# olof3/QuantumOptimalControl.jl

Hardware: AMD Instinct MI355X
Metric: GRAPE gradient evals/sec (dim N, T slices, B seeds) @ 1/2/4/8 GPU (higher is better)
Workload: dtype f64

## Files before the change

quantumoptimalcontrol.jl_amd/csrc/qoc_blkseg.hpp:

```cpp
#pragma once
#include "qoc_blku.hpp"

namespace qoc {

struct BlksegParams {
  double rad[3];
  double mur[3], mui[3];
  double theta_cap;
  int S;
  int L;
  int UPW;
  int RB;
  const double* u;
  double* u_copy;
  double* u_copy2;
  double* J2;
  cx<double>* coef2;
  double* dJdu;
  unsigned long long* terms;
  unsigned int* done;
  double* best;
  long long seed_offset;
  double* best_res;
  double* best_out;
  double2* gseg;
  const int* stale;
  const double2* gtab;
  double pen_mu;
  unsigned int prow[3];
  unsigned int pcol;
  double2* dseg;
};
enum { BLKSEG_FUSED = 0, BLKSEG_FWD = 1, BLKSEG_BWD = 2 };

__host__ __device__ inline size_t blkseg_off_rec(int NB, int nblk) { return (size_t)6 * NB * NB * nblk; }
__host__ __device__ inline size_t blkseg_off_slot(int NB, int nblk, int Nt) { return blkseg_off_rec(NB, nblk) + 4 * (size_t)Nt; }
__host__ __device__ inline size_t blkseg_off_g0(int NB, int nblk, int Nt, int S) {
  return blkseg_off_slot(NB, nblk, Nt) + (size_t)2 * S * NB * NB * nblk;
}
__host__ __device__ inline size_t blkseg_off_xN(int NB, int nblk, int Nt, int S) {
  return blkseg_off_g0(NB, nblk, Nt, S) + (size_t)2 * NB * NB * nblk;
}
__host__ __device__ inline size_t blkseg_off_xt(int N, int m, int NB, int nblk, int Nt, int S) {
  return blkseg_off_xN(NB, nblk, Nt, S) + (size_t)2 * N * m;
}
__host__ __device__ inline size_t blkseg_off_cf(int N, int m, int NB, int nblk, int Nt, int S) {
  return blkseg_off_xt(N, m, NB, nblk, Nt, S) + (size_t)2 * N * m;
}
__host__ __device__ inline size_t blkseg_off_red(int N, int m, int NB, int nblk, int Nt, int S) {
  return blkseg_off_cf(N, m, NB, nblk, Nt, S) + (size_t)4 * m;
}
__host__ __device__ inline size_t blkseg_off_wred(int N, int m, int NB, int nblk, int Nt, int S) {
  return blkseg_off_red(N, m, NB, nblk, Nt, S) + 32;
}
__host__ __device__ inline size_t blkseg_off_dJ(int N, int m, int NB, int nblk, int Nt, int S, int W, int RB) {
  return blkseg_off_wred(N, m, NB, nblk, Nt, S) + (size_t)128 * W * RB;
}
__host__ __device__ inline size_t blkseg_off_d0(int N, int m, int nu, int NB, int nblk, int Nt, int S, int W, int RB) {
  return (blkseg_off_dJ(N, m, NB, nblk, Nt, S, W, RB) + (size_t)Nt * nu + 1) & ~(size_t)1;
}
__host__ __device__ inline size_t blkseg_lds(int N, int m, int nu, int NB, int nblk, int Nt, int S, int W, int RB,
                                             bool pen = false) {
  if (pen) return (blkseg_off_d0(N, m, nu, NB, nblk, Nt, S, W, RB) + (size_t)2 * NB * NB * nblk) * sizeof(double);
  return (blkseg_off_dJ(N, m, NB, nblk, Nt, S, W, RB) + (size_t)Nt * nu) * sizeof(double);
}
constexpr size_t BLKSEG_LDS_MAX = (size_t)160 * 1024;
__host__ __device__ inline int blkseg_rb(int upw, int nu) {
  const int r = 64 / (upw * (nu > 0 ? nu : 1));
  return r < 1 ? 1 : r > 4 ? 4 : r;
}

#ifdef QOC_PROBE
static __device__ unsigned long long g_segw[32];
#define SEGW_SET(slot, v)                                                        \
  do {                                                                           \
    if (blockIdx.x == 7 && (threadIdx.x & 63) == 0) g_segw[slot] = (v);          \
  } while (0)
static __device__ int g_seg_noturn, g_seg_turnmode;
#define SEG_TURNS (!g_seg_noturn)
#define SEG_TURNMODE g_seg_turnmode
#else
#define SEG_TURNS true
#define SEG_TURNMODE 1
#define SEGW_SET(slot, v) \
  do {                    \
  } while (0)
#endif


template <int NB, bool AH, bool BH>
__device__ __forceinline__ void seg_mm(const double (&ar)[NB * NB], const double (&ai)[NB * NB], const double (&br)[NB * NB],
                                       const double (&bi)[NB * NB], double (&cr)[NB * NB], double (&ci)[NB * NB]) {
#pragma unroll
  for (int i = 0; i < NB; ++i)
#pragma unroll
    for (int k = 0; k < NB; ++k) {
      double sr = 0.0, si = 0.0;
#pragma unroll
      for (int q = 0; q < NB; ++q) {
        const int ea = AH ? q * NB + i : i * NB + q, eb = BH ? k * NB + q : q * NB + k;
// ... 207 lines not shown
#pragma unroll
  for (int k = K - 1; k >= 0; --k) {
    ct = fma(ct, t2, T.c[k]);
    st = fma(st, t2, T.s[k]);
  }
  st *= t;
}
template <int K = BLKSEG_KMAX>
__device__ __forceinline__ void sk2_z(const Sk2& g0, const double* rec, double& zr, double& zi) {
  double ct, st;
  sk2_phase<K>(g0.d0, g0.d1, ct, st);
  const double2 ph = *reinterpret_cast<const double2*>(rec);
  zr = ph.x * ct - ph.y * st;
  zi = fma(ph.x, st, ph.y * ct);
}
template <int K = BLKSEG_KMAX, bool EX = false>
__device__ __forceinline__ void sk2_form(const Sk2 (&g)[3], double2 ph, double2 u, Sk2& ah, double (&ur)[4],
                                         double (&ui)[4], double* ex = nullptr) {
  constexpr BlksegTrig T = blkseg_trig();
  ah.d0 = fma(u.y, g[2].d0, fma(u.x, g[1].d0, g[0].d0));
  ah.d1 = fma(u.y, g[2].d1, fma(u.x, g[1].d1, g[0].d1));
  ah.r = fma(u.y, g[2].r, fma(u.x, g[1].r, g[0].r));
  ah.q = fma(u.y, g[2].q, fma(u.x, g[1].q, g[0].q));
  const double a = 0.5 * (ah.d0 - ah.d1);
  const double w = fma(a, a, fma(ah.r, ah.r, ah.q * ah.q));
  double cw = T.c[K], sw = T.s[K], s3 = EX ? T.d[K] : 0.0, ct, st;
#pragma unroll
  for (int k = K - 1; k >= 0; --k) {
    cw = fma(cw, w, T.c[k]);
    sw = fma(sw, w, T.s[k]);
// ... 385 lines not shown
  constexpr int NV1 = NB == 2 ? 2 : 1;
  const int N = g.N, m = g.m, nu = g.nu, Nt = g.Nt, nblk = bk.nblk, S = sp.S, L = sp.L;
  const int tid = threadIdx.x, nthr = blockDim.x, w = tid >> 6, l = tid & 63, W = nthr >> 6;
  const int b = blockIdx.x;
  const size_t Nm = (size_t)N * m;
  BK_T(t0);
  double* const lds = reinterpret_cast<double*>(smem);
  double2* const gsh = reinterpret_cast<double2*>(lds);
  double* const rec = lds + blkseg_off_rec(NB, nblk);
  double2* const slot = reinterpret_cast<double2*>(lds + blkseg_off_slot(NB, nblk, Nt));
  double2* const g0s = reinterpret_cast<double2*>(lds + blkseg_off_g0(NB, nblk, Nt, S));
  double* const xN = lds + blkseg_off_xN(NB, nblk, Nt, S);
  double2* const xtl = reinterpret_cast<double2*>(lds + blkseg_off_xt(N, m, NB, nblk, Nt, S));
  cx<double>* const cf = reinterpret_cast<cx<double>*>(lds + blkseg_off_cf(N, m, NB, nblk, Nt, S));
  double* const red = lds + blkseg_off_red(N, m, NB, nblk, Nt, S);
  double* const wred = lds + blkseg_off_wred(N, m, NB, nblk, Nt, S);
  const int RB = sp.RB;
  double* const dJ = lds + blkseg_off_dJ(N, m, NB, nblk, Nt, S, W, RB);
  double2* const d0s = reinterpret_cast<double2*>(lds + blkseg_off_d0(N, m, nu, NB, nblk, Nt, S, W, RB));

  const int uw = l / nblk;
  const bool lact = uw < sp.UPW;
  const int beta = lact ? l - uw * nblk : 0;
  int pm = 0;
  if constexpr (PEN) {
    if (lact && w * sp.UPW + uw < S)
#pragma unroll
      for (int i = 0; i < NB; ++i) pm |= (int)((sp.prow[i] >> beta) & 1u) << i;
  }
  constexpr int PE = PEN ? NB * NB : 1;
  const int ntab = 3 * E * nblk;
  const double2* const x0g = reinterpret_cast<const double2*>(g.x0) + (g.x0_per_seed ? (size_t)b * Nm : 0);
  const double2* const xtg = reinterpret_cast<const double2*>(g.Xt);
  const double* ub = sp.u + (size_t)b * Nt * nu;
  const bool u16 = nu == 2 && (reinterpret_cast<size_t>(ub) & 15) == 0;
  auto load_u = [&](int k) -> double2 {
    if (u16) return reinterpret_cast<const double2*>(ub)[k];
    return make_double2(nu > 0 ? ub[(size_t)k * nu] : 0.0, nu > 1 ? ub[(size_t)k * nu + 1] : 0.0);
  };
  const bool hasx = MODE != BLKSEG_BWD && (size_t)tid < Nm;
  double2 tab0 = make_double2(0.0, 0.0), x00 = tab0, xt0 = tab0, ua = tab0, ubb = tab0;
  if (tid < ntab) tab0 = sp.gtab[tid];
  if (hasx) {
    x00 = x0g[tid];
    xt0 = xtg[tid];
  }
  if (tid < Nt) ua = load_u(tid);
  if (tid + nthr < Nt) ubb = load_u(tid + nthr);
  int brw[NB];
#pragma unroll
  for (int i = 0; i < NB; ++i) brw[i] = bk.brow[beta * NB + i];
  {
    if (tid < ntab) gsh[tid] = tab0;
    for (int q = tid + nthr; q < ntab; q += nthr) gsh[q] = sp.gtab[q];
    if constexpr (MODE != BLKSEG_BWD) {
      double2* const xN2 = reinterpret_cast<double2*>(xN);
      if (hasx) {
        xN2[tid] = x00;
        xtl[tid] = xt0;
      }
      for (size_t o = (size_t)tid + nthr; o < Nm; o += nthr) {
        xN2[o] = x0g[o];
        xtl[o] = xtg[o];
      }
    }
  }
  double rmax = 0.0;
  const bool cmu = sp.mur[1] == 0.0 && sp.mur[2] == 0.0 && sp.mui[1] == 0.0 && sp.mui[2] == 0.0;
  double2 emu0 = make_double2(1.0, 0.0);
  if (cmu) {
    const double er = exp(sp.mur[0]);
    double sn, cs;
    sincos(sp.mui[0], &sn, &cs);
    emu0 = make_double2(er * cs, er * sn);
  }
  auto slice = [&](int k, double2 uk) {
    const double u1 = uk.x, u2 = uk.y;
    for (int j = 0; j < nu; ++j) {
      const double v = j ? u2 : u1;
      if (sp.u_copy) sp.u_copy[((size_t)b * Nt + k) * nu + j] = v;
      if (sp.u_copy2) sp.u_copy2[((size_t)b * Nt + k) * nu + j] = v;
    }
    rmax = fmax(rmax, fma(fabs(u2), sp.rad[2], fma(fabs(u1), sp.rad[1], sp.rad[0])));
    double2* r = reinterpret_cast<double2*>(rec + 4 * (size_t)k);
    if (cmu) {
      r[0] = emu0;
    } else {
      const double mr = fma(u2, sp.mur[2], fma(u1, sp.mur[1], sp.mur[0]));
      const double mi = fma(u2, sp.mui[2], fma(u1, sp.mui[1], sp.mui[0]));
      const double er = exp(mr);
      double sn, cs;
      sincos(mi, &sn, &cs);
      r[0] = make_double2(er * cs, er * sn);
    }
    r[1] = make_double2(u1, u2);
  };
  if (tid < Nt) slice(tid, ua);
  if (tid + nthr < Nt) slice(tid + nthr, ubb);
  for (int k = tid + 2 * nthr; k < Nt; k += nthr) slice(k, load_u(k));
  rmax = block_max(rmax, red);
  int J = 0;
  double s0 = 1.0;
  while (rmax * s0 > sp.theta_cap && J < 60) {
    s0 *= 0.5;
    ++J;
  }
  int P = 0;
  {
    const double bb = rmax * s0, tol = 1.1102230246251565e-16;
    constexpr BlkuCoef K = blku_coef();
    double term = bb;
#pragma unroll
    for (int q = 0; q < BLKU_TMAX; ++q) {
      if (!(term > tol * fma(-bb, K.inv[q + 2], 1.0))) break;
      P = q + 1;
      term *= bb * K.inv[q + 2];
    }
  }
  P = __builtin_amdgcn_readfirstlane(P);
  J = __builtin_amdgcn_readfirstlane(J);
  int nex = 1;
  if constexpr (ORD == 0) nex = __builtin_amdgcn_readfirstlane(blkseg_exact_terms(rmax));
  if (tid < 8) reinterpret_cast<int*>(red + 24)[tid] = 0;
  if (J) {
    for (int k = tid; k < Nt; k += nthr) {
      rec[4 * (size_t)k + 2] *= s0;
      rec[4 * (size_t)k + 3] *= s0;
    }
  }
  __syncthreads();
  BK_T(t1);
  BK_ADD(0, t1 - t0);

  const int s = w * sp.UPW + uw;
  const bool sact = lact && s < S;
  const int kb = sact ? s * L : 0;
  const int ke = sact ? min(kb + L, Nt) : 0;
  double2 greg[GREG ? 3 : 1][GREG ? E : 1];
  if constexpr (GREG) {
#pragma unroll
    for (int j = 0; j < 3; ++j)
#pragma unroll
      for (int e = 0; e < E; ++e) greg[j][e] = gsh[(beta * 3 + j) * E + e];
  }
  auto gen_at = [&](int bc) {
    return [&, bc](int j, int e) -> double2 {
// ... 23 lines not shown
  double Hr[PE], Hi[PE];
#pragma unroll
  for (int e = 0; e < PE; ++e) Hr[e] = Hi[e] = 0.0;
  const int Lf = Nt - (S - 1) * L;
  const bool fast = NB == 2 && J == 0;
  Sk2 gk[3];
  if constexpr (NB == 2) {
#pragma unroll
    for (int j = 0; j < 3; ++j) {
      double2 e4[4];
#pragma unroll
      for (int e = 0; e < 4; ++e) e4[e] = gsh[(beta * 3 + j) * E + e];
      gk[j] = sk2_of(e4);
    }
  }
  const bool zdl = NB != 2 || (gk[1].d0 == 0.0 && gk[1].d1 == 0.0 && gk[2].d0 == 0.0 && gk[2].d1 == 0.0);
  const bool zd = __syncthreads_and(zdl ? 1 : 0) != 0 && cmu && sp.mur[0] == 0.0;
  const double za0 = NB == 2 ? 0.5 * (gk[0].d0 - gk[0].d1) : 0.0;
  const int ksel = __builtin_amdgcn_readfirstlane(blkseg_series_k(rmax * s0));
  const bool su = fast && zd;
  double pq[4] = {1.0, 0.0, 0.0, 0.0};
  auto lane_z = [&](double& zr, double& zi) {
    zr = 1.0;
    zi = 0.0;
    if constexpr (NB == 2) {
      if (su) {
        if (ksel == 5) sk2_z<5>(gk[0], rec, zr, zi);
        else if (ksel == 7) sk2_z<7>(gk[0], rec, zr, zi);
        else sk2_z<BLKSEG_KMAX>(gk[0], rec, zr, zi);
      }
    }
  };
  const double* const reck = rec + 4 * (size_t)kb;
  auto p1_fast = [&](int jj, auto SEL_, auto K_, auto ZD_) {
    constexpr bool SEL = decltype(SEL_)::value;
    constexpr int KS = decltype(K_)::value;
    constexpr bool ZD = decltype(ZD_)::value;
    if constexpr (NB == 2) {
    if constexpr (ZD) {
      double vv[2][4];
      bool act[2];
#pragma unroll
      for (int v = 0; v < 2; ++v) {
        const int k = kb + jj + v;
// ... 168 lines not shown
      ti[e] = v.y;
    }
    wave_lds_sync();
    if (take) {
      double cr[E], ci[E];
      seg_mm<NB, false, false>(qr, qi, tr, ti, cr, ci);
#pragma unroll
      for (int e = 0; e < E; ++e) {
        qr[e] = cr[e];
        qi[e] = ci[e];
        slot_at(s, e) = make_double2(cr[e], ci[e]);
      }
    }
    wave_lds_sync();
  }
  lds_barrier();
  if (sact && w > 0) {
    double er[E], ei[E];
#pragma unroll
    for (int e = 0; e < E; ++e) {
      const double2 v = slot_at(UPW - 1, e);
      er[e] = v.x;
      ei[e] = v.y;
    }
    for (int v = 1; v < w; ++v) {
      double tr[E], ti[E], cr[E], ci[E];
#pragma unroll
      for (int e = 0; e < E; ++e) {
        const double2 x = slot_at(v * UPW + UPW - 1, e);
        tr[e] = x.x;
        ti[e] = x.y;
      }
      seg_mm<NB, false, false>(tr, ti, er, ei, cr, ci);
#pragma unroll
      for (int e = 0; e < E; ++e) {
        er[e] = cr[e];
        ei[e] = ci[e];
      }
    }
    double cr[E], ci[E];
    seg_mm<NB, false, false>(qr, qi, er, ei, cr, ci);
#pragma unroll
    for (int e = 0; e < E; ++e) {
      qr[e] = cr[e];
      qi[e] = ci[e];
    }
  }
  if constexpr (PEN) {
    if (pm) {
      double tr[E], ti[E];
      seg_mm<NB, true, false>(qr, qi, Hr, Hi, tr, ti);
      seg_mm<NB, false, false>(tr, ti, qr, qi, Hr, Hi);
    }
  }
  const bool last = sact && s == S - 1;
  if (last) {
    double znr = 1.0, zni = 0.0;
    if (su) {
      double br, bi;
      lane_z(br, bi);
      for (int n = Nt; n > 0; n >>= 1) {
        if (n & 1) {
          const double t = znr * br - zni * bi;
          zni = fma(znr, bi, zni * br);
          znr = t;
        }
        const double t = br * br - bi * bi;
        bi = 2.0 * (br * bi);
        br = t;
      }
    }
    for (int c = 0; c < m; ++c) {
      double xr[NB], xi[NB];
#pragma unroll
      for (int i = 0; i < NB; ++i) {
        const size_t o = 2 * ((size_t)c * N + max(brw[i], 0));
        xr[i] = brw[i] >= 0 ? xN[o] : 0.0;
        xi[i] = brw[i] >= 0 ? xN[o + 1] : 0.0;
      }
#pragma unroll
      for (int i = 0; i < NB; ++i) {
        double yr = 0.0, yi = 0.0;
#pragma unroll
        for (int q = 0; q < NB; ++q) {
          yr = fma(qr[i * NB + q], xr[q], fma(-qi[i * NB + q], xi[q], yr));
          yi = fma(qr[i * NB + q], xi[q], fma(qi[i * NB + q], xr[q], yi));
        }
        if (su) {
          const double t = yr * znr - yi * zni;
          yi = fma(yr, zni, yi * znr);
          yr = t;
        }
        if (brw[i] >= 0) {
          const size_t o = 2 * ((size_t)c * N + brw[i]);
          xN[o] = yr;
          xN[o + 1] = yi;
        }
      }
    }
  }
  __syncthreads();
  if constexpr (PEN) {
    if (pm)
#pragma unroll
      for (int e = 0; e < E; ++e) slot_at(s, e) = make_double2(Hr[e], Hi[e]);
    wave_lds_sync();
    for (int d = 1; d < UPW; d <<= 1) {
      const bool take = pm && uw0 + d < UPW && s + d < S;
      double tr[E], ti[E];
#pragma unroll
      for (int e = 0; e < E; ++e) {
        const double2 v = take ? slot_at(s + d, e) : make_double2(0.0, 0.0);
        tr[e] = v.x;
        ti[e] = v.y;
      }
      wave_lds_sync();
// ... 48 lines not shown
  }
  if (tid == 0) {
    double Jv = red[16];
    if constexpr (PEN) {
      double ps = 0.0;
      for (int q = 0; q < nblk; ++q) ps += wred[q];
      Jv = fma(sp.pen_mu, ps, Jv);
    }
    __hip_atomic_store(reinterpret_cast<unsigned long long*>(g.J + b),
                       (unsigned long long)__double_as_longlong(Jv), __ATOMIC_RELAXED, __HIP_MEMORY_SCOPE_AGENT);
    if (sp.J2) sp.J2[b] = Jv;
  }
#if defined(__HIP_DEVICE_COMPILE__) && !defined(__gfx950__)
#error "k_blkseg_eval's best-(J, seed) hand-off is written for gfx950"
#endif
  const bool early = W <= 4;
  auto publish = [&]() {
    if (w != 0 || !sp.done) return;
    unsigned int prev = 0;
    if (l == 0) {
      asm volatile("s_waitcnt vmcnt(0)" ::: "memory");
      prev = __hip_atomic_fetch_add(sp.done, 1u, __ATOMIC_RELAXED, __HIP_MEMORY_SCOPE_AGENT);
    }
    prev = __shfl(prev, 0);
    if (prev == gridDim.x - 1) {
      __builtin_amdgcn_fence(__ATOMIC_ACQUIRE, "agent");
      asm volatile("s_waitcnt vmcnt(0)" ::: "memory");
      double bv = __builtin_inf();
      long long bi = -1;
      for (int e = l; e < (int)gridDim.x; e += 64) {
// ... 52 lines not shown
#pragma unroll
    for (int e = 0; e < E; ++e) g0s[e * nblk + beta] = make_double2(cr[e], ci[e]);
  }
  if constexpr (PEN) {
    if (pm) {
      later_waves(Hr, Hi);
      if (uw0 + 1 < UPW && s + 1 < S)
#pragma unroll
        for (int e = 0; e < E; ++e) {
          const double2 x = slot_at(s + 1, e);
          Hr[e] += x.x;
          Hi[e] += x.y;
        }
    }
  }
  __syncthreads();
  {
    double hr[E], hi[E], tr[E], ti[E];
#pragma unroll
    for (int e = 0; e < E; ++e) {
      const double2 v = g0s[e * nblk + beta];
      hr[e] = v.x;
      hi[e] = v.y;
    }
    if constexpr (PEN) {
      if (pm) {
        double dr[E], di[E];
#pragma unroll
        for (int e = 0; e < E; ++e) {
          const double2 v = d0s[e * nblk + beta];
          dr[e] = v.x;
// ... 23 lines not shown
#pragma unroll
            for (int q = 0; q < NB; ++q) {
              sr = fma(dr[i * NB + q], Hr[q * NB + j], fma(-di[i * NB + q], Hi[q * NB + j], sr));
              si = fma(dr[i * NB + q], Hi[q * NB + j], fma(di[i * NB + q], Hr[q * NB + j], si));
            }
            hr[i * NB + j] = fma(f, sr, hr[i * NB + j]);
            hi[i * NB + j] = fma(f, si, hi[i * NB + j]);
          }
        __builtin_amdgcn_sched_barrier(0);
      }
    }
    seg_mm<NB, false, false>(qr, qi, hr, hi, tr, ti);
    seg_mm<NB, false, true>(tr, ti, qr, qi, Gr, Gi);
  }

  if (!early) publish();
  BK_T(t2e);
  BK_ADD(2, t2e - t2);
  if constexpr (MODE == BLKSEG_FWD) {
    if (sact)
#pragma unroll
      for (int e = 0; e < E; ++e) gseg_at(e) = make_double2(Gr[e], Gi[e]);
    if (sp.terms && tid == 0) atomicAdd(sp.terms + b % TERM_SLOTS, (unsigned long long)Nt * ((unsigned long long)P << J));
    return;
  }
  }
  BK_T(t3);
  const double mu1r = sp.mur[1], mu1i = sp.mui[1], mu2r = sp.mur[2], mu2i = sp.mui[2];
  const double pen2 = PEN ? 2.0 * sp.pen_mu : 0.0;
  auto pen_step = [&](const double (&ur)[E], const double (&ui)[E]) {
    seg_pen_step<NB>(pm, pen2, slot + (size_t)opaque(s) * E * nblk + beta, nblk, ur, ui, Gr, Gi);
  };
  double zr, zi;
  lane_z(zr, zi);
  if (su) {
#pragma unroll
    for (int e = 0; e < E; ++e) {
      const double t = fma(zr, Gr[e], zi * Gi[e]);
      Gi[e] = fma(zr, Gi[e], -zi * Gr[e]);
      Gr[e] = t;
    }
  }
  const double pen2r = pen2 * zr, pen2i = -pen2 * zi;
  auto pen_step_v = [&](const double (&ur)[E], const double (&ui)[E]) {
    seg_pen_step<NB, true>(pm, pen2r, slot + (size_t)opaque(s) * E * nblk + beta, nblk, ur, ui, Gr, Gi, pen2i);
  };
  double* const wr = wred + 128 * RB * w;
  const int nrl = sp.UPW * max(nu, 1);
  const int rq = l / nrl, rrem = l - rq * nrl, ro = rrem / max(nu, 1), rj = rrem - ro * max(nu, 1);
  int rslot = 0;
  auto reduce = [&](int jj, double acc1, double acc2) {
    const int r = rslot;
    rslot = r == RB - 1 ? 0 : r + 1;
    *reinterpret_cast<double2*>(wr + 128 * r + 2 * l) = make_double2(acc1, acc2);
    if (r == RB - 1 || jj == 0) {
      wave_lds_sync();
      if (rq <= r) {
        const int ss = w * sp.UPW + ro, kk = ss * L + jj + r - rq;
        if (ss < S && kk < Nt) {
          const double* src = wr + 128 * rq + 2 * ro * nblk + rj;
          double sum = 0.0;
          for (int q = 0; q < nblk; ++q) sum += src[2 * q];
          dJ[(size_t)kk * nu + rj] = sum;
        }
      }
      wave_lds_sync();
    }
  };
  double pa1[4] = {0, 0, 0, 0}, pa2[4] = {0, 0, 0, 0};
  const double zxd0 = NB == 2 ? gk[0].d0 + sp.mui[0] : 0.0, zxd1 = NB == 2 ? gk[0].d1 + sp.mui[0] : 0.0;
  const double zx0 = 0.5 * (zxd0 + zxd1), zx3 = 0.5 * (zxd0 - zxd1), zx02 = zx0 * zx0;
  if constexpr (NB == 2) {
    sk2_pauli2(Sk2{gk[1].d0 + mu1i, gk[1].d1 + mu1i, gk[1].r, gk[1].q}, pa1);
    sk2_pauli2(Sk2{gk[2].d0 + mu2i, gk[2].d1 + mu2i, gk[2].r, gk[2].q}, pa2);
  }
  auto p3_fast = [&](int jj, auto SEL_, auto K_, auto ZD_, const double2* upre = nullptr) {
    constexpr bool SEL = decltype(SEL_)::value;
    constexpr int KS = decltype(K_)::value;
// ... 130 lines not shown
        const double2* const gp = slot + (size_t)opaque(sact ? s : 0) * E * nblk + beta;
#pragma unroll
        for (int e = 0; e < E; ++e) {
          const double2 v = gp[e * nblk];
          Gr[e] = v.x;
          Gi[e] = v.y;
        }
      }
      reduce(jj, act ? acc1 : 0.0, act ? acc2 : 0.0);
    }
  }
  if (turns || sprog.on) __builtin_amdgcn_s_setprio(0);
  BK_T(t4);
  BK_ADD(3, t4 - t3);
  SEGW_SET(16 + w, t4 - t0);
  __syncthreads();
  double* const og = sp.dJdu + (size_t)b * Nt * nu;
  for (int i = tid; i < Nt * nu; i += nthr) og[i] = dJ[i];
  if (MODE == BLKSEG_FUSED && sp.terms && tid == 0)
    atomicAdd(sp.terms + b % TERM_SLOTS, (unsigned long long)Nt * ((unsigned long long)P << J));
  BK_T(t5);
  BK_ADD(4, t5 - t4);
  BK_ADD(5, t5 - t0);
}

}
```

quantumoptimalcontrol.jl_amd/csrc/qoc_engine.hip:

```cpp
#include <dlfcn.h>

#include "qoc_internal.hpp"
#include "qoc_spline.hpp"
#include "qoc_opt.hpp"

namespace qoc_host {

thread_local std::string g_err;

int fail(qoc_ctx* ctx, int code, const char* fmt, ...) {
  char buf[512];
  va_list ap;
  va_start(ap, fmt);
  vsnprintf(buf, sizeof(buf), fmt, ap);
  va_end(ap);
  g_err = buf;
  if (ctx) ctx->err = buf;
  return code;
}

template <typename T>
int upload_complex(qoc_ctx* ctx, const double* host, void* dev, size_t nelem) {
  if (sizeof(T) == sizeof(double)) {
    HIPCHK(ctx, hipMemcpyAsync(dev, host, nelem * 16, hipMemcpyHostToDevice, ctx->stream));
// ... 483 lines not shown
  *out = c;
  return QOC_OK;
}

void qoc_destroy(qoc_ctx* c) {
  if (!c) return;
  hipSetDevice(c->dev);
  if (c->stream) hipStreamSynchronize(c->stream);
  if (c->comm && rccl().commDestroy) rccl().commDestroy(c->comm);
  if (c->d_best) hipFree(c->d_best);
  if (c->d_done) hipFree(c->d_done);
  if (c->d_tcoef) hipFree(c->d_tcoef);
  if (c->d_coef_mu) hipFree(c->d_coef_mu);
  if (c->d_brow) hipFree(c->d_brow);
  if (c->d_gtab) hipFree(c->d_gtab);
  if (c->d_wrow) hipFree(c->d_wrow);
  if (c->d_wrow_live) hipFree(c->d_wrow_live);
  if (c->d_dead_rows) hipFree(c->d_dead_rows);
  if (c->d_gc_part) hipFree(c->d_gc_part);
  if (c->d_gseg) hipFree(c->d_gseg);
  if (c->d_blkp_ctab) hipFree(c->d_blkp_ctab);
  if (c->d_blkp_M) hipFree(c->d_blkp_M);
  if (c->d_blkp_ph) hipFree(c->d_blkp_ph);
  if (c->d_minmax) hipFree(c->d_minmax);
  if (c->h_minmax) hipHostFree(c->h_minmax);
  if (c->h_flag) hipHostFree(c->h_flag);
  if (c->flag_ev) hipEventDestroy(c->flag_ev);
  void* ptrs[] = {c->d_A, c->d_x0, c->d_Xt, c->d_pmask, c->d_u,    c->d_U,    c->d_X, c->d_L, c->d_u_lam, c->d_coef_lam, c->d_blkU, c->d_J_scr, c->d_coef_scr,
                  c->d_J, c->d_coef, c->d_dJdu, c->d_flag, c->d_hist, c->d_stage, c->d_ws, c->d_red, c->d_Bs, c->d_cstage, c->d_fws, c->d_AH, c->d_Cst, c->d_gws, c->d_pws, c->d_ps, c->d_At, c->d_steps, c->d_terms, c->d_src, c->d_rsec, c->d_sink, c->d_blkrec, c->d_xn};
  for (void* p : ptrs)
// ... 1271 lines not shown
```

quantumoptimalcontrol.jl_amd/csrc/qoc_internal.hpp:

```cpp
#pragma once
#include <hip/hip_runtime.h>

#include <algorithm>
#include <cmath>
#include <cstdarg>
#include <cstdio>
#include <cstdlib>
#include <cstring>
#include <initializer_list>
#include <string>
#include <type_traits>
#include <vector>

#include "../../include/qoc.h"
#include "qoc_chain.hpp"
#include "qoc_comm.hpp"
#include "qoc_tchain.hpp"

namespace qoc {
struct BlkArgs;
}
using namespace qoc;

struct BlksegShape {
// ... 141 lines not shown
  mutable unsigned int seg_prow[3] = {0, 0, 0}, seg_pcol = 0;
  std::vector<int> h_brow;
  int* h_flag = nullptr;
  int flag_turn = 0;
  hipEvent_t flag_ev = nullptr;
  double* d_J_scr = nullptr;
  cx<double>* d_coef_scr = nullptr;
  bool skew_exact = false;
  cx<double>* d_coef_lam = nullptr;
  cx<double>* d_coef_mu = nullptr;
  int last_eval_mode = 0;
  int blk_nb = 0;
  int nblk = 0;
  int* d_brow = nullptr;
  double2* d_gtab = nullptr;
  int blk_jr = 0;
  bool blk_real = false;
  int nwb = 0;
  int* d_wrow = nullptr;
  std::vector<int> h_wrow;
  std::vector<int> h_wrow_live, h_dead_rows;
  double* d_gc_part = nullptr;
  size_t gc_part_bytes = 0;
  std::vector<int> h_dead_zeroed;
  const void* dead_bufs[6] = {};
  bool dead_dirty = true;
  int* d_wrow_live = nullptr;
  int* d_dead_rows = nullptr;
  size_t blk_dev_bytes = 0;
  double* d_blkrec = nullptr;
// ... 141 lines not shown
int blkp_pen_mode(const qoc_ctx* c);
bool blkp_fits_nwb(const qoc_ctx* c, int nwb);
bool blkp_exact_on(const qoc_ctx* c);
int blkp_eval_concurrent(qoc_ctx* c, int order, double* d_dJdu, const BlkArgs& bk);
int blkp_forward(qoc_ctx* c);
bool blkp_backward_ok(const qoc_ctx* c, int order);
int blkp_backward(qoc_ctx* c, int order, double* d_dJdu, const int* stale);

int blku_forward(qoc_ctx* c);
int blku_backward(qoc_ctx* c, int order, double* d_dJdu);
int blku_eval_concurrent(qoc_ctx* c, int order, double* d_dJdu);
int blku_states(qoc_ctx* c);
int blku_costates(qoc_ctx* c);

bool blkseg_ok(const qoc_ctx* c, int order);
int blkseg_eval(qoc_ctx* c, int order, const double* d_u, double* d_J, double* d_dJdu);
bool blkseg_split_ok(const qoc_ctx* c);
int blkseg_forward(qoc_ctx* c, const double* d_u, double* d_J);
int blkseg_backward(qoc_ctx* c, int order, double* d_dJdu, const int* stale);

}
```

quantumoptimalcontrol.jl_amd/csrc/qoc_run_blk.hip:

```cpp
#include <numeric>

#include "qoc_blk_host.hpp"

namespace qoc_host {

int blk_detect(qoc_ctx* c) {
  c->blk_nb = 0;
  c->nblk = 0;
  c->blk_jr = 0;
  c->blk_real = false;
  c->nwb = 0;
  c->h_brow.clear();
  c->seg_pen_valid = false;
  if (env_is("QOC_BLOCKS", "0")) return QOC_OK;
  const bool valu = env_is("QOC_BLOCKS", "valu");
  const bool real_req = env_is("QOC_BLOCKS", "real");
  const int N = c->N;
  const size_t NN = (size_t)N * N;
  std::vector<int> par(N);
  std::iota(par.begin(), par.end(), 0);
  auto find = [&](int x) {
    while (par[x] != x) x = par[x] = par[par[x]];
    return x;
  };
// ... 85 lines not shown
    const int E = NB * NB;
    std::vector<double> tab((size_t)nblk * 3 * E * 2, 0.0);
    for (int b = 0; b < nblk; ++b)
      for (int j = 0; j <= c->nu && j < 3; ++j)
        for (int e = 0; e < E; ++e) {
          const int ri = brow[(size_t)b * NB + e / NB], rk = brow[(size_t)b * NB + e % NB];
          if (ri < 0 || rk < 0) continue;
          const double* v = c->h_gen.data() + 2 * (j * NN + ri + (size_t)N * rk);
          double* t = tab.data() + 2 * (((size_t)b * 3 + j) * E + e);
          t[0] = ri == rk ? v[0] - c->tprm.mur[j] : v[0];
          t[1] = ri == rk ? v[1] - c->tprm.mui[j] : v[1];
        }
    HIPCHK(c, hipMalloc((void**)&c->d_gtab, tab.size() * sizeof(double)));
    HIPCHK(c, hipMemcpy(c->d_gtab, tab.data(), tab.size() * sizeof(double), hipMemcpyHostToDevice));
    c->blk_dev_bytes += tab.size() * sizeof(double);
  }
  if (jr || real) {
    HIPCHK(c, hipMalloc((void**)&c->d_wrow, wrow.size() * sizeof(int)));
    HIPCHK(c, hipMemcpy(c->d_wrow, wrow.data(), wrow.size() * sizeof(int), hipMemcpyHostToDevice));
    c->blk_dev_bytes += wrow.size() * sizeof(int);
  }
  c->dev_bytes += c->blk_dev_bytes;
  c->blk_nb = NB;
  c->nblk = nblk;
  c->blk_jr = jr;
  c->blk_real = real;
  c->nwb = (int)(wrow.size() / 16);
  return QOC_OK;
}

bool blk_active(const qoc_ctx* c) {
  if (c->blk_nb <= 0 || c->prec != QOC_FP64 || c->chain_mode != 1 || c->prop_method != QOC_PROP_EXPM || c->big ||
      c->packed || c->nu > 2)
    return false;
  if (c->blk_real) return c->nwb * ((c->m + 3) / 4) <= 8;
  if (c->blk_jr) return c->nwb * ((c->m + 1) / 2) <= 8 && (c->blk_nb < 16 || tchain_mf(c));
  return c->nblk * c->m <= BLK_MAXT && c->nblk <= 256;
}
bool blk_rot(const qoc_ctx* c) { return c->blk_jr > 0 || c->blk_real; }

bool blku_on(const qoc_ctx* c) {
  if (!blk_active(c) || c->blk_jr != 1 || c->blk_nb > BLK_NBMAX || c->nu < 1 || c->nu > 2 || c->nblk > 32 ||
// ... 249 lines not shown
```

quantumoptimalcontrol.jl_amd/csrc/qoc_run_blkseg.hip:

```cpp
#include <cstring>

#include "qoc_blk_host.hpp"
#include "qoc_blkseg.hpp"
#include "qoc_internal.hpp"

namespace qoc_host {

static bool blkseg_pen(const qoc_ctx* c) {
  if (c->mu == 0.0) return false;
  if (!c->seg_pen_valid) {
    c->seg_prow[0] = c->seg_prow[1] = c->seg_prow[2] = 0;
    c->seg_pcol = 0;
    const int NB = c->blk_nb;
    if (NB >= 2 && NB <= 3 && c->nblk <= 32 && (int)c->h_brow.size() == c->nblk * NB)
      for (int r : c->h_pen_rows)
        for (int q = 0; q < c->nblk * NB; ++q)
          if (c->h_brow[q] == r) c->seg_prow[q % NB] |= 1u << (q / NB);
    for (int col : c->h_pen_cols)
      if (col >= 0 && col < 32) c->seg_pcol |= 1u << col;
    c->seg_pen_valid = true;
  }
  return (c->seg_prow[0] | c->seg_prow[1] | c->seg_prow[2]) != 0 && c->seg_pcol != 0;
}

// ... 35 lines not shown
}

template <typename F>
static hipError_t blkseg_dispatch(int NB, int order, F&& f) {
  if (order == QOC_DUKDP_EXACT) {
    const std::integral_constant<int, 0> ex;
    if (NB == 2) return f(std::integral_constant<int, 2>(), ex);
    return f(std::integral_constant<int, 3>(), ex);
  }
  return blk_order_dispatch(order, [&](auto ORD_) {
    if (NB == 2) return f(std::integral_constant<int, 2>(), ORD_);
    return f(std::integral_constant<int, 3>(), ORD_);
  });
}

static int ensure_lazy_bufs(qoc_ctx* c) {
  const size_t nu_t = (size_t)c->B * c->nu * c->Nt, ncf = (size_t)c->B * 2 * c->m_user;
  if (!c->d_u_lam) {
    HIPCHK(c, hipMalloc((void**)&c->d_u_lam, nu_t * sizeof(double)));
    HIPCHK(c, hipMalloc((void**)&c->d_coef_lam, ncf * sizeof(cx<double>)));
    c->dev_bytes += nu_t * sizeof(double) + ncf * sizeof(cx<double>);
  }
  return QOC_OK;
}

static int blkseg_params(qoc_ctx* c, const BlksegShape& s, BlksegParams& sp) {
  sp = BlksegParams{};
  for (int j = 0; j < 3; ++j) {
    const bool on = j <= c->nu;
    sp.rad[j] = on ? c->tprm.rad[j] : 0.0;
    sp.mur[j] = on ? c->tprm.mur[j] : 0.0;
    sp.mui[j] = on ? c->tprm.mui[j] : 0.0;
  }
  sp.theta_cap = c->tprm.theta[17];
  sp.S = s.S;
  sp.L = s.L;
  sp.UPW = s.UPW;
  sp.RB = s.RB;
  sp.gtab = c->d_gtab;
  sp.terms = c->d_terms;
  if (blkseg_pen(c)) {
    sp.pen_mu = c->mu;
    for (int i = 0; i < 3; ++i) sp.prow[i] = c->seg_prow[i];
    sp.pcol = c->seg_pcol;
  }
  if (!c->d_best) {
    HIPCHK(c, hipMalloc((void**)&c->d_best, 6 * sizeof(double)));
    c->world = 1;
// ... 152 lines not shown
```

Before: 4.821 million.

## Precompute per-block phase constants on host setup and trim blkseg LDS staging

Adds a one-block setup kernel that precomputes, per diagonal block, the drift phase z for each series order and its Nt-th power, plus exp(mu0). The main kernel reads these from LDS instead of re-evaluating the phase series and doing a repeated-squaring power per lane. It also moves the zero-drift check to the host, writes dJdu straight to global memory without the LDS staging buffer and final copy loop, and for NB=2 preloads and unrolls the cross-wave segment product chain. The cost is an extra cached device table that must be invalidated correctly when gtab, Nt or mu change, plus probe timing macros.

After: 4.766 million. 1.2% lower.

```diff
diff --git a/quantumoptimalcontrol.jl_amd/csrc/qoc_blkseg.hpp b/quantumoptimalcontrol.jl_amd/csrc/qoc_blkseg.hpp
--- a/quantumoptimalcontrol.jl_amd/csrc/qoc_blkseg.hpp
+++ b/quantumoptimalcontrol.jl_amd/csrc/qoc_blkseg.hpp
@@ -26,6 +26,8 @@
   double2* gseg;
   const int* stale;
   const double2* gtab;
+  const double2* ctab;
+  int zd;
   double pen_mu;
   unsigned int prow[3];
   unsigned int pcol;
@@ -50,19 +52,20 @@
 __host__ __device__ inline size_t blkseg_off_red(int N, int m, int NB, int nblk, int Nt, int S) {
   return blkseg_off_cf(N, m, NB, nblk, Nt, S) + (size_t)4 * m;
 }
+__host__ __device__ inline size_t blkseg_off_zt(int N, int m, int NB, int nblk, int Nt, int S) {
+  return blkseg_off_red(N, m, NB, nblk, Nt, S) + 32;
+}
+__host__ __device__ inline int blkseg_nzt(int NB, int nblk) { return NB == 2 ? 6 * nblk : 0; }
 __host__ __device__ inline size_t blkseg_off_wred(int N, int m, int NB, int nblk, int Nt, int S) {
-  return blkseg_off_red(N, m, NB, nblk, Nt, S) + 32;
-}
-__host__ __device__ inline size_t blkseg_off_dJ(int N, int m, int NB, int nblk, int Nt, int S, int W, int RB) {
+  return blkseg_off_zt(N, m, NB, nblk, Nt, S) + (size_t)2 * blkseg_nzt(NB, nblk);
+}
+__host__ __device__ inline size_t blkseg_off_d0(int N, int m, int NB, int nblk, int Nt, int S, int W, int RB) {
   return blkseg_off_wred(N, m, NB, nblk, Nt, S) + (size_t)128 * W * RB;
-}
-__host__ __device__ inline size_t blkseg_off_d0(int N, int m, int nu, int NB, int nblk, int Nt, int S, int W, int RB) {
-  return (blkseg_off_dJ(N, m, NB, nblk, Nt, S, W, RB) + (size_t)Nt * nu + 1) & ~(size_t)1;
 }
 __host__ __device__ inline size_t blkseg_lds(int N, int m, int nu, int NB, int nblk, int Nt, int S, int W, int RB,
                                              bool pen = false) {
-  if (pen) return (blkseg_off_d0(N, m, nu, NB, nblk, Nt, S, W, RB) + (size_t)2 * NB * NB * nblk) * sizeof(double);
-  return (blkseg_off_dJ(N, m, NB, nblk, Nt, S, W, RB) + (size_t)Nt * nu) * sizeof(double);
+  (void)nu;
+  return (blkseg_off_d0(N, m, NB, nblk, Nt, S, W, RB) + (pen ? (size_t)2 * NB * NB * nblk : 0)) * sizeof(double);
 }
 constexpr size_t BLKSEG_LDS_MAX = (size_t)160 * 1024;
 __host__ __device__ inline int blkseg_rb(int upw, int nu) {
@@ -75,6 +78,11 @@
 #define SEGW_SET(slot, v)                                                        \
   do {                                                                           \
     if (blockIdx.x == 7 && (threadIdx.x & 63) == 0) g_segw[slot] = (v);          \
+  } while (0)
+static __device__ unsigned long long g_bks[32];
+#define BKS_ADD(slot, v)                                                          \
+  do {                                                                            \
+    if (blockIdx.x == 7 && (threadIdx.x & 63) == 0) atomicAdd(&g_bks[slot], (v)); \
   } while (0)
 static __device__ int g_seg_noturn, g_seg_turnmode;
 #define SEG_TURNS (!g_seg_noturn)
@@ -84,6 +92,9 @@
 #define SEG_TURNMODE 1
 #define SEGW_SET(slot, v) \
   do {                    \
+  } while (0)
+#define BKS_ADD(slot, v) \
+  do {                   \
   } while (0)
 #endif
 
@@ -321,6 +332,51 @@
   zr = ph.x * ct - ph.y * st;
   zi = fma(ph.x, st, ph.y * ct);
 }
+__device__ __forceinline__ void sk2_zpow(double br, double bi, int n, double& znr, double& zni) {
+  znr = 1.0;
+  zni = 0.0;
+  for (; n > 0; n >>= 1) {
+    if (n & 1) {
+      const double t = znr * br - zni * bi;
+      zni = fma(znr, bi, zni * br);
+      znr = t;
+    }
+    const double t = br * br - bi * bi;
+    bi = 2.0 * (br * bi);
+    br = t;
+  }
+}
+__device__ __forceinline__ double2 seg_emu0(double mur0, double mui0) {
+  const double er = exp(mur0);
+  double sn, cs;
+  sincos(mui0, &sn, &cs);
+  return make_double2(er * cs, er * sn);
+}
+static __global__ void k_blkseg_consts(const double2* __restrict__ gtab, int NB, int nblk, int Nt, int cmu,
+                                       double mur0, double mui0, double2* __restrict__ ctab) {
+  const double2 emu0 = cmu ? seg_emu0(mur0, mui0) : make_double2(1.0, 0.0);
+  if (threadIdx.x == 0) ctab[0] = emu0;
+  if (NB != 2) return;
+  alignas(16) const double ph[2] = {emu0.x, emu0.y};
+  for (int beta = threadIdx.x; beta < nblk; beta += blockDim.x) {
+    double2 e4[4];
+#pragma unroll
+    for (int e = 0; e < 4; ++e) e4[e] = gtab[(beta * 3 + 0) * 4 + e];
+    const Sk2 g0 = sk2_of(e4);
+    double zr[3], zi[3];
+    sk2_z<5>(g0, ph, zr[0], zi[0]);
+    sk2_z<7>(g0, ph, zr[1], zi[1]);
+    sk2_z<BLKSEG_KMAX>(g0, ph, zr[2], zi[2]);
+#pragma unroll
+    for (int c = 0; c < 3; ++c) {
+      double nr, ni;
+      sk2_zpow(zr[c], zi[c], Nt, nr, ni);
+      ctab[1 + 2 * (c * nblk + beta)] = make_double2(zr[c], zi[c]);
+      ctab[2 + 2 * (c * nblk + beta)] = make_double2(nr, ni);
+    }
+  }
+}
+
 template <int K = BLKSEG_KMAX, bool EX = false>
 __device__ __forceinline__ void sk2_form(const Sk2 (&g)[3], double2 ph, double2 u, Sk2& ah, double (&ur)[4],
                                          double (&ui)[4], double* ex = nullptr) {
@@ -736,10 +792,10 @@
   double2* const xtl = reinterpret_cast<double2*>(lds + blkseg_off_xt(N, m, NB, nblk, Nt, S));
   cx<double>* const cf = reinterpret_cast<cx<double>*>(lds + blkseg_off_cf(N, m, NB, nblk, Nt, S));
   double* const red = lds + blkseg_off_red(N, m, NB, nblk, Nt, S);
+  double2* const zts = reinterpret_cast<double2*>(lds + blkseg_off_zt(N, m, NB, nblk, Nt, S));
   double* const wred = lds + blkseg_off_wred(N, m, NB, nblk, Nt, S);
   const int RB = sp.RB;
-  double* const dJ = lds + blkseg_off_dJ(N, m, NB, nblk, Nt, S, W, RB);
-  double2* const d0s = reinterpret_cast<double2*>(lds + blkseg_off_d0(N, m, nu, NB, nblk, Nt, S, W, RB));
+  double2* const d0s = reinterpret_cast<double2*>(lds + blkseg_off_d0(N, m, NB, nblk, Nt, S, W, RB));
 
   const int uw = l / nblk;
   const bool lact = uw < sp.UPW;
@@ -761,8 +817,13 @@
     return make_double2(nu > 0 ? ub[(size_t)k * nu] : 0.0, nu > 1 ? ub[(size_t)k * nu + 1] : 0.0);
   };
   const bool hasx = MODE != BLKSEG_BWD && (size_t)tid < Nm;
-  double2 tab0 = make_double2(0.0, 0.0), x00 = tab0, xt0 = tab0, ua = tab0, ubb = tab0;
+  double2 tab0 = make_double2(0.0, 0.0), x00 = tab0, xt0 = tab0, ua = tab0, ubb = tab0, zt0 = tab0;
   if (tid < ntab) tab0 = sp.gtab[tid];
+  const int nzt = sp.zd ? blkseg_nzt(NB, nblk) : 0;
+  if (tid < nzt) zt0 = sp.ctab[1 + tid];
+  const bool cmu = sp.mur[1] == 0.0 && sp.mur[2] == 0.0 && sp.mui[1] == 0.0 && sp.mui[2] == 0.0;
+  double2 emu0 = make_double2(1.0, 0.0);
+  if (cmu) emu0 = sp.ctab[0];
   if (hasx) {
     x00 = x0g[tid];
     xt0 = xtg[tid];
@@ -772,9 +833,13 @@
   int brw[NB];
 #pragma unroll
   for (int i = 0; i < NB; ++i) brw[i] = bk.brow[beta * NB + i];
+  BK_T(pa);
+  BKS_ADD(0, pa - t0);
   {
     if (tid < ntab) gsh[tid] = tab0;
     for (int q = tid + nthr; q < ntab; q += nthr) gsh[q] = sp.gtab[q];
+    if (tid < nzt) zts[tid] = zt0;
+    for (int q = tid + nthr; q < nzt; q += nthr) zts[q] = sp.ctab[1 + q];
     if constexpr (MODE != BLKSEG_BWD) {
       double2* const xN2 = reinterpret_cast<double2*>(xN);
       if (hasx) {
@@ -787,15 +852,11 @@
       }
     }
   }
+  BK_T(pb);
+  BKS_ADD(1, pb - pa);
   double rmax = 0.0;
-  const bool cmu = sp.mur[1] == 0.0 && sp.mur[2] == 0.0 && sp.mui[1] == 0.0 && sp.mui[2] == 0.0;
-  double2 emu0 = make_double2(1.0, 0.0);
-  if (cmu) {
-    const double er = exp(sp.mur[0]);
-    double sn, cs;
-    sincos(sp.mui[0], &sn, &cs);
-    emu0 = make_double2(er * cs, er * sn);
-  }
+  BK_T(pc);
+  BKS_ADD(2, pc - pb);
   auto slice = [&](int k, double2 uk) {
     const double u1 = uk.x, u2 = uk.y;
     for (int j = 0; j < nu; ++j) {
@@ -820,7 +881,12 @@
   if (tid < Nt) slice(tid, ua);
   if (tid + nthr < Nt) slice(tid + nthr, ubb);
   for (int k = tid + 2 * nthr; k < Nt; k += nthr) slice(k, load_u(k));
+  BK_T(pd);
+  BKS_ADD(3, pd - pc);
   rmax = block_max(rmax, red);
+  if (tid < 8) reinterpret_cast<int*>(red + 24)[tid] = 0;
+  BK_T(pe);
+  BKS_ADD(4, pe - pd);
   int J = 0;
   double s0 = 1.0;
   while (rmax * s0 > sp.theta_cap && J < 60) {
@@ -843,7 +909,8 @@
   J = __builtin_amdgcn_readfirstlane(J);
   int nex = 1;
   if constexpr (ORD == 0) nex = __builtin_amdgcn_readfirstlane(blkseg_exact_terms(rmax));
-  if (tid < 8) reinterpret_cast<int*>(red + 24)[tid] = 0;
+  BK_T(pf);
+  BKS_ADD(5, pf - pe);
   if (J) {
     for (int k = tid; k < Nt; k += nthr) {
       rec[4 * (size_t)k + 2] *= s0;
@@ -852,6 +919,7 @@
   }
   __syncthreads();
   BK_T(t1);
+  BKS_ADD(6, t1 - pf);
   BK_ADD(0, t1 - t0);
 
   const int s = w * sp.UPW + uw;
@@ -905,20 +973,20 @@
       gk[j] = sk2_of(e4);
     }
   }
-  const bool zdl = NB != 2 || (gk[1].d0 == 0.0 && gk[1].d1 == 0.0 && gk[2].d0 == 0.0 && gk[2].d1 == 0.0);
-  const bool zd = __syncthreads_and(zdl ? 1 : 0) != 0 && cmu && sp.mur[0] == 0.0;
+  const bool zd = sp.zd != 0;
   const double za0 = NB == 2 ? 0.5 * (gk[0].d0 - gk[0].d1) : 0.0;
   const int ksel = __builtin_amdgcn_readfirstlane(blkseg_series_k(rmax * s0));
   const bool su = fast && zd;
   double pq[4] = {1.0, 0.0, 0.0, 0.0};
-  auto lane_z = [&](double& zr, double& zi) {
+  const double2* const ztl = zts + 2 * ((ksel == 5 ? 0 : ksel == 7 ? 1 : 2) * nblk + beta);
+  auto lane_z = [&](double& zr, double& zi, int pw) {
     zr = 1.0;
     zi = 0.0;
     if constexpr (NB == 2) {
       if (su) {
-        if (ksel == 5) sk2_z<5>(gk[0], rec, zr, zi);
-        else if (ksel == 7) sk2_z<7>(gk[0], rec, zr, zi);
-        else sk2_z<BLKSEG_KMAX>(gk[0], rec, zr, zi);
+        const double2 z = ztl[pw];
+        zr = z.x;
+        zi = z.y;
       }
     }
   };
@@ -1117,7 +1185,11 @@
     }
     wave_lds_sync();
   }
+  BK_T(qa);
+  BKS_ADD(8, qa - t2);
   lds_barrier();
+  BK_T(qb);
+  BKS_ADD(9, qb - qa);
   if (sact && w > 0) {
     double er[E], ei[E];
 #pragma unroll
@@ -1126,19 +1198,43 @@
       er[e] = v.x;
       ei[e] = v.y;
     }
-    for (int v = 1; v < w; ++v) {
-      double tr[E], ti[E], cr[E], ci[E];
-#pragma unroll
-      for (int e = 0; e < E; ++e) {
-        const double2 x = slot_at(v * UPW + UPW - 1, e);
-        tr[e] = x.x;
-        ti[e] = x.y;
-      }
-      seg_mm<NB, false, false>(tr, ti, er, ei, cr, ci);
-#pragma unroll
-      for (int e = 0; e < E; ++e) {
-        er[e] = cr[e];
-        ei[e] = ci[e];
+    if constexpr (NB == 2) {
+      double tr[WMAX - 2][E], ti[WMAX - 2][E];
+#pragma unroll
+      for (int v = 1; v < WMAX - 1; ++v)
+        if (v < w)
+#pragma unroll
+          for (int e = 0; e < E; ++e) {
+            const double2 x = slot_at(v * UPW + UPW - 1, e);
+            tr[v - 1][e] = x.x;
+            ti[v - 1][e] = x.y;
+          }
+#pragma unroll
+      for (int v = 1; v < WMAX - 1; ++v)
+        if (v < w) {
+          double cr[E], ci[E];
+          seg_mm<NB, false, false>(tr[v - 1], ti[v - 1], er, ei, cr, ci);
+#pragma unroll
+          for (int e = 0; e < E; ++e) {
+            er[e] = cr[e];
+            ei[e] = ci[e];
+          }
+        }
+    } else {
+      for (int v = 1; v < w; ++v) {
+        double tr[E], ti[E], cr[E], ci[E];
+#pragma unroll
+        for (int e = 0; e < E; ++e) {
+          const double2 x = slot_at(v * UPW + UPW - 1, e);
+          tr[e] = x.x;
+          ti[e] = x.y;
+        }
+        seg_mm<NB, false, false>(tr, ti, er, ei, cr, ci);
+#pragma unroll
+        for (int e = 0; e < E; ++e) {
+          er[e] = cr[e];
+          ei[e] = ci[e];
+        }
       }
     }
     double cr[E], ci[E];
@@ -1156,23 +1252,12 @@
       seg_mm<NB, false, false>(tr, ti, qr, qi, Hr, Hi);
     }
   }
+  BK_T(qc);
+  BKS_ADD(10, qc - qb);
   const bool last = sact && s == S - 1;
   if (last) {
-    double znr = 1.0, zni = 0.0;
-    if (su) {
-      double br, bi;
-      lane_z(br, bi);
-      for (int n = Nt; n > 0; n >>= 1) {
-        if (n & 1) {
-          const double t = znr * br - zni * bi;
-          zni = fma(znr, bi, zni * br);
-          znr = t;
-        }
-        const double t = br * br - bi * bi;
-        bi = 2.0 * (br * bi);
-        br = t;
-      }
-    }
+    double znr, zni;
+    lane_z(znr, zni, 1);
     for (int c = 0; c < m; ++c) {
       double xr[NB], xi[NB];
 #pragma unroll
@@ -1202,7 +1287,11 @@
       }
     }
   }
+  BK_T(qd);
+  BKS_ADD(11, qd - qc);
   __syncthreads();
+  BK_T(qe);
+  BKS_ADD(12, qe - qd);
   if constexpr (PEN) {
     if (pm)
 #pragma unroll
@@ -1281,6 +1370,8 @@
 #if defined(__HIP_DEVICE_COMPILE__) && !defined(__gfx950__)
 #error "k_blkseg_eval's best-(J, seed) hand-off is written for gfx950"
 #endif
+  BK_T(qf);
+  BKS_ADD(13, qf - qe);
   const bool early = W <= 4;
   auto publish = [&]() {
     if (w != 0 || !sp.done) return;
@@ -1363,7 +1454,11 @@
         }
     }
   }
+  BK_T(qg);
+  BKS_ADD(14, qg - qf);
   __syncthreads();
+  BK_T(qh);
+  BKS_ADD(15, qh - qg);
   {
     double hr[E], hi[E], tr[E], ti[E];
 #pragma unroll
@@ -1417,8 +1512,11 @@
     seg_mm<NB, false, true>(tr, ti, qr, qi, Gr, Gi);
   }
 
+  BK_T(qi);
+  BKS_ADD(16, qi - qh);
   if (!early) publish();
   BK_T(t2e);
+  BKS_ADD(17, t2e - qi);
   BK_ADD(2, t2e - t2);
   if constexpr (MODE == BLKSEG_FWD) {
     if (sact)
@@ -1435,7 +1533,7 @@
     seg_pen_step<NB>(pm, pen2, slot + (size_t)opaque(s) * E * nblk + beta, nblk, ur, ui, Gr, Gi);
   };
   double zr, zi;
-  lane_z(zr, zi);
+  lane_z(zr, zi, 0);
   if (su) {
 #pragma unroll
     for (int e = 0; e < E; ++e) {
@@ -1449,6 +1547,7 @@
     seg_pen_step<NB, true>(pm, pen2r, slot + (size_t)opaque(s) * E * nblk + beta, nblk, ur, ui, Gr, Gi, pen2i);
   };
   double* const wr = wred + 128 * RB * w;
+  double* const og = sp.dJdu + (size_t)b * Nt * nu;
   const int nrl = sp.UPW * max(nu, 1);
   const int rq = l / nrl, rrem = l - rq * nrl, ro = rrem / max(nu, 1), rj = rrem - ro * max(nu, 1);
   int rslot = 0;
@@ -1464,7 +1563,7 @@
           const double* src = wr + 128 * rq + 2 * ro * nblk + rj;
           double sum = 0.0;
           for (int q = 0; q < nblk; ++q) sum += src[2 * q];
-          dJ[(size_t)kk * nu + rj] = sum;
+          og[(size_t)kk * nu + rj] = sum;
         }
       }
       wave_lds_sync();
@@ -1625,9 +1724,6 @@
   BK_T(t4);
   BK_ADD(3, t4 - t3);
   SEGW_SET(16 + w, t4 - t0);
-  __syncthreads();
-  double* const og = sp.dJdu + (size_t)b * Nt * nu;
-  for (int i = tid; i < Nt * nu; i += nthr) og[i] = dJ[i];
   if (MODE == BLKSEG_FUSED && sp.terms && tid == 0)
     atomicAdd(sp.terms + b % TERM_SLOTS, (unsigned long long)Nt * ((unsigned long long)P << J));
   BK_T(t5);
diff --git a/quantumoptimalcontrol.jl_amd/csrc/qoc_engine.hip b/quantumoptimalcontrol.jl_amd/csrc/qoc_engine.hip
--- a/quantumoptimalcontrol.jl_amd/csrc/qoc_engine.hip
+++ b/quantumoptimalcontrol.jl_amd/csrc/qoc_engine.hip
@@ -521,6 +521,7 @@
   if (c->d_coef_mu) hipFree(c->d_coef_mu);
   if (c->d_brow) hipFree(c->d_brow);
   if (c->d_gtab) hipFree(c->d_gtab);
+  if (c->d_segc) hipFree(c->d_segc);
   if (c->d_wrow) hipFree(c->d_wrow);
   if (c->d_wrow_live) hipFree(c->d_wrow_live);
   if (c->d_dead_rows) hipFree(c->d_dead_rows);
diff --git a/quantumoptimalcontrol.jl_amd/csrc/qoc_internal.hpp b/quantumoptimalcontrol.jl_amd/csrc/qoc_internal.hpp
--- a/quantumoptimalcontrol.jl_amd/csrc/qoc_internal.hpp
+++ b/quantumoptimalcontrol.jl_amd/csrc/qoc_internal.hpp
@@ -179,6 +179,12 @@
   int nblk = 0;
   int* d_brow = nullptr;
   double2* d_gtab = nullptr;
+  std::vector<double> h_gtab;
+  int gtab_gen = 0;
+  double2* d_segc = nullptr;
+  size_t segc_n = 0;
+  double segc_key[10] = {-1, -1, -1, -1, 0, 0, 0, 0, 0, 0};
+  int seg_zd = 0;
   int blk_jr = 0;
   bool blk_real = false;
   int nwb = 0;
@@ -350,6 +356,7 @@
 int blku_costates(qoc_ctx* c);
 
 bool blkseg_ok(const qoc_ctx* c, int order);
+int blkseg_consts(qoc_ctx* c);
 int blkseg_eval(qoc_ctx* c, int order, const double* d_u, double* d_J, double* d_dJdu);
 bool blkseg_split_ok(const qoc_ctx* c);
 int blkseg_forward(qoc_ctx* c, const double* d_u, double* d_J);
diff --git a/quantumoptimalcontrol.jl_amd/csrc/qoc_run_blk.hip b/quantumoptimalcontrol.jl_amd/csrc/qoc_run_blk.hip
--- a/quantumoptimalcontrol.jl_amd/csrc/qoc_run_blk.hip
+++ b/quantumoptimalcontrol.jl_amd/csrc/qoc_run_blk.hip
@@ -123,6 +123,8 @@
     HIPCHK(c, hipMalloc((void**)&c->d_gtab, tab.size() * sizeof(double)));
     HIPCHK(c, hipMemcpy(c->d_gtab, tab.data(), tab.size() * sizeof(double), hipMemcpyHostToDevice));
     c->blk_dev_bytes += tab.size() * sizeof(double);
+    c->h_gtab = std::move(tab);
+    c->gtab_gen++;
   }
   if (jr || real) {
     HIPCHK(c, hipMalloc((void**)&c->d_wrow, wrow.size() * sizeof(int)));
@@ -135,6 +137,7 @@
   c->blk_jr = jr;
   c->blk_real = real;
   c->nwb = (int)(wrow.size() / 16);
+  if (NB <= 3) return blkseg_consts(c);
   return QOC_OK;
 }
 
diff --git a/quantumoptimalcontrol.jl_amd/csrc/qoc_run_blkseg.hip b/quantumoptimalcontrol.jl_amd/csrc/qoc_run_blkseg.hip
--- a/quantumoptimalcontrol.jl_amd/csrc/qoc_run_blkseg.hip
+++ b/quantumoptimalcontrol.jl_amd/csrc/qoc_run_blkseg.hip
@@ -73,6 +73,51 @@
   });
 }
 
+static void blkseg_shifts(const qoc_ctx* c, double (&mur)[3], double (&mui)[3]) {
+  for (int j = 0; j < 3; ++j) {
+    const bool on = j <= c->nu;
+    mur[j] = on ? c->tprm.mur[j] : 0.0;
+    mui[j] = on ? c->tprm.mui[j] : 0.0;
+  }
+}
+
+int blkseg_consts(qoc_ctx* c) {
+  const int NB = c->blk_nb, nblk = c->nblk;
+  if ((NB != 2 && NB != 3) || !c->d_gtab) return QOC_OK;
+  double mur[3], mui[3];
+  blkseg_shifts(c, mur, mui);
+  const double key[10] = {(double)c->gtab_gen, (double)NB, (double)nblk, (double)c->Nt, mur[0], mur[1], mur[2],
+                          mui[0], mui[1], mui[2]};
+  if (c->d_segc && std::memcmp(key, c->segc_key, sizeof(key)) == 0) return QOC_OK;
+  const size_t n = 1 + (size_t)blkseg_nzt(NB, nblk);
+  if (c->segc_n < n) {
+    if (c->d_segc) {
+      HIPCHK(c, hipFree(c->d_segc));
+      c->d_segc = nullptr;
+      c->dev_bytes -= c->segc_n * sizeof(double2);
+      c->segc_n = 0;
+    }
+    HIPCHK(c, hipMalloc((void**)&c->d_segc, n * sizeof(double2)));
+    c->segc_n = n;
+    c->dev_bytes += n * sizeof(double2);
+  }
+  const bool cmu = mur[1] == 0.0 && mur[2] == 0.0 && mui[1] == 0.0 && mui[2] == 0.0;
+  bool zdl = true;
+  if (NB == 2 && c->h_gtab.size() == (size_t)nblk * 3 * 4 * 2)
+    for (int b = 0; b < nblk; ++b)
+      for (int j = 1; j < 3; ++j) {
+        const double* t = c->h_gtab.data() + 2 * ((size_t)b * 3 + j) * 4;
+        zdl = zdl && t[1] == 0.0 && t[7] == 0.0;
+      }
+  c->seg_zd = zdl && cmu && mur[0] == 0.0 ? 1 : 0;
+  hipLaunchKernelGGL(k_blkseg_consts, dim3(1), dim3(64), 0, c->stream, c->d_gtab, NB, nblk, c->Nt, cmu ? 1 : 0, mur[0],
+                     mui[0], c->d_segc);
+  const hipError_t e = hipGetLastError();
+  if (e != hipSuccess) return fail(c, QOC_ERR_HIP, "k_blkseg_consts launch: %s", hipGetErrorString(e));
+  std::memcpy(c->segc_key, key, sizeof(key));
+  return QOC_OK;
+}
+
 static int ensure_lazy_bufs(qoc_ctx* c) {
   const size_t nu_t = (size_t)c->B * c->nu * c->Nt, ncf = (size_t)c->B * 2 * c->m_user;
   if (!c->d_u_lam) {
@@ -85,12 +130,12 @@
 
 static int blkseg_params(qoc_ctx* c, const BlksegShape& s, BlksegParams& sp) {
   sp = BlksegParams{};
-  for (int j = 0; j < 3; ++j) {
-    const bool on = j <= c->nu;
-    sp.rad[j] = on ? c->tprm.rad[j] : 0.0;
-    sp.mur[j] = on ? c->tprm.mur[j] : 0.0;
-    sp.mui[j] = on ? c->tprm.mui[j] : 0.0;
-  }
+  for (int j = 0; j < 3; ++j) sp.rad[j] = j <= c->nu ? c->tprm.rad[j] : 0.0;
+  blkseg_shifts(c, sp.mur, sp.mui);
+  const int rc = blkseg_consts(c);
+  if (rc) return rc;
+  sp.ctab = c->d_segc;
+  sp.zd = c->seg_zd;
   sp.theta_cap = c->tprm.theta[17];
   sp.S = s.S;
   sp.L = s.L;
```
